# crowsonkb/style_transfer2

Measured on AMD Instinct MI355X. Metric: style-transfer iters/sec @1024px VGG19, higher is better.
Workload: dtype f32; 1 GPU; configs[1]: 1024x1024 single image per GPU, VGG19 to conv5_1, content conv4_2 + 5 style layers, adam fp32, 500 iterations per image; jobs=1, parallelism=independent jobs, 1 per GPU, no collective (replicas)

## Files before the change

### style_transfer2_amd/csrc/conv3x3_winograd.hip

```cpp
#include <hip/hip_runtime.h>
#include <stdint.h>
#include <stdlib.h>
#include <string.h>
#include <type_traits>
#include "st2_kernels.h"
#include "env.h"

namespace st2 {

typedef float f32x16 __attribute__((ext_vector_type(16)));
typedef float f32x4 __attribute__((ext_vector_type(4)));


constexpr int WN_CH = 8;
constexpr int WN_IW = 40;
constexpr int WN_V = 4 * 16 * 64;

size_t wino_pack_floats(int K, int M) { return (size_t)((M + 127) / 128 * 4) * (K / 2) * 1024; }

static void wino_pack(const float* w, int Cout, int Cin, bool dgrad, float* dst)
{
    const int K = dgrad ? Cout : Cin, M = dgrad ? Cin : Cout, nkp = K / 2;
    memset(dst, 0, wino_pack_floats(K, M) * sizeof(float));
    static const double G[4][3] = {{1, 0, 0}, {0.5, 0.5, 0.5}, {0.5, -0.5, 0.5}, {0, 0, 1}};
    for (int m = 0; m < M; ++m)
        for (int k = 0; k < K; ++k) {
            double g[3][3], t[4][3], u[4][4];
            for (int tap = 0; tap < 9; ++tap)
                g[tap / 3][tap % 3] = dgrad ? w[((size_t)k * Cin + m) * 9 + (8 - tap)] : w[((size_t)m * Cin + k) * 9 + tap];
            for (int i = 0; i < 4; ++i)
                for (int j = 0; j < 3; ++j) t[i][j] = G[i][0] * g[0][j] + G[i][1] * g[1][j] + G[i][2] * g[2][j];
            for (int i = 0; i < 4; ++i)
                for (int j = 0; j < 4; ++j) u[i][j] = t[i][0] * G[j][0] + t[i][1] * G[j][1] + t[i][2] * G[j][2];
            const size_t base = ((size_t)(m / 32) * nkp + k / 2) * 1024;
            const int lane = (k & 1) * 32 + (m & 31);
            for (int pos = 0; pos < 16; ++pos)
                dst[base + ((size_t)(pos >> 2) * 64 + lane) * 4 + (pos & 3)] = (float)u[pos >> 2][pos & 3];
        }
}
void pack_wino_weights_fwd(const float* w, int Cout, int Cin, float* dst) { wino_pack(w, Cout, Cin, false, dst); }
void pack_wino_weights_dgrad(const float* w, int Cout, int Cin, float* dst) { wino_pack(w, Cout, Cin, true, dst); }

struct WinoKArgs {
    const float* in; const float4* upack; const float* bias; float* out;
    const float* mask_src; const float* inject;
    int K, M, H, W, nch, tiles_x, tiles_y, n_mtiles, relu;
    unsigned in_bytes, u_bytes;
    float* pool_out; int pool_h, pool_w;
    unsigned char* pool_amap;
    const unsigned char* unpool_amap; unsigned amap_bytes; int ph, pw;
    int splits; float* scratch;
    unsigned long long* stamps;
};

typedef __attribute__((address_space(3))) void* lptr_t;
constexpr unsigned kOOB = 0xffffffffu;

__device__ __forceinline__ float f4c(const float4& v, int i) { return i == 0 ? v.x : i == 1 ? v.y : i == 2 ? v.z : v.w; }

template <int WM, int TG, int DIAG = 0, bool QUAD = true, bool PS = false, bool W8 = false, bool H4 = false, bool UNPOOL = false, bool BIG = false,
          bool NOOUT = false, int EPI = 0>
__device__ __forceinline__ void conv3x3_wino_body(const WinoKArgs& a)
{
    static_assert(EPI == 0 || (QUAD && TG == 1 && !PS && !W8 && !BIG && DIAG == 0), "specialised epilogues: aligned widths, one tile group, four waves, below 4 GiB");
    static_assert(!NOOUT || EPI == 0 || EPI == 2, "no-output builds pool");
    static_assert(!NOOUT || (QUAD && TG == 1 && !PS && !W8 && !UNPOOL && !BIG && DIAG == 0), "no-output builds: the builds that write the arg-max map");
    static_assert(!BIG || (QUAD && TG == 1 && !PS && !W8 && DIAG == 0), "big tensors: aligned widths, one tile group, four waves");
    static_assert(!UNPOOL || (QUAD && TG == 1 && !PS && !W8), "unpool: aligned widths, one tile group, four waves");
    static_assert(H4 || (WM * TG == 4 && (TG == 1 || TG == 2)), "4 waves");
    static_assert(!PS || (WM == 2 && TG == 2), "position split: 2 channel slices x 2 position halves");
    static_assert(!W8 || (WM == 4 && TG == 1 && QUAD && !PS), "eight waves: 4 channel slices x 2 position halves, aligned widths");
    static_assert(!H4 || (WM == 2 && TG == 1 && QUAD && !PS && !W8), "half tile: 2 channel slices x 2 position halves, aligned widths");
    constexpr bool RS = W8 || H4;
    constexpr bool AMAP = QUAD && TG == 1;
    constexpr int NW = W8 ? 8 : 4;
    constexpr int PARTNER = W8 ? 4 : 2;
    constexpr bool SPLIT = PS || RS;
    constexpr int BM = 32 * WM;
    constexpr int PROWS = 4 * TG;
    constexpr int IN_ROWS = PROWS + 2;
    constexpr int IW = QUAD ? WN_IW : 64;
    constexpr int COL0 = QUAD ? 3 : 0;
    constexpr int PLANE = IN_ROWS * IW;
    constexpr int UP_ROWS = PROWS / 2 + 2, UP_COLS = 24;
    constexpr int UP_PLANE = UP_ROWS * UP_COLS;
    constexpr int UP_F = WN_CH * UP_PLANE;
    constexpr int UP_FQ = UP_F / 256, UP_AQ = UP_F / 256;
    static_assert(!UNPOOL || (UP_F % 256 == 0 && NW == 4), "unpool staging is a whole number of wave-DMAs");
    constexpr int N_RAW = UNPOOL ? UP_F + UP_F / 4 : WN_CH * PLANE;
    constexpr int I_PER_WAVE = UNPOOL ? (UP_FQ + UP_AQ + NW - 1) / NW
                             : QUAD ? (N_RAW / 4 + 64 * NW - 1) / (64 * NW) : WN_CH * IN_ROWS / 4;
    constexpr int RAW = UNPOOL ? 1024 : QUAD ? I_PER_WAVE * NW * 256 : N_RAW;
    static_assert(QUAD || (WN_CH * IN_ROWS) % 4 == 0, "rows divide over the four waves");

    __shared__ __attribute__((aligned(16))) float raw_s[2][RAW];
    __shared__ __attribute__((aligned(16))) float v_s[2][TG][WN_V];
    __shared__ __attribute__((aligned(16))) float x8_own[W8 ? 8 * 8 * 64 * 4 : 4];
    static_assert(!H4 || 4 * 8 * 64 * 4 <= 2 * TG * WN_V, "H4: the exchange buffer fits the V images");
    float* const x8_s = H4 ? &v_s[0][0][0] : x8_own;

    const int tid = threadIdx.x;
    const int lane = tid & 63;
    const int wave = __builtin_amdgcn_readfirstlane(tid >> 6);
    const int wave_m = W8 ? (wave & 3) : H4 ? (wave & 1) : wave / TG, wave_g = RS ? 0 : wave % TG;
    const int ph = W8 ? wave >> 2 : H4 ? wave >> 1 : wave_g;

    const int nwg = gridDim.x / a.splits;
    const int split = blockIdx.x / nwg, orig = blockIdx.x - split * nwg;
    const int nch = a.nch / a.splits, c_first = split * nch;
    const int xcd = orig & 7, q = nwg >> 3, r = nwg & 7;
    const int logical = (xcd < r ? xcd * (q + 1) : r * (q + 1) + (xcd - r) * q) + (orig >> 3);
    const int n_pt = a.tiles_x * a.tiles_y;
    const int mt = logical / n_pt;
    const int pt = logical - mt * n_pt;
    const int tx = pt % a.tiles_x;
    const int ty = pt / a.tiles_x;
    const int y0 = ty * PROWS, x0 = tx * 32;
    const unsigned plane = (unsigned)a.H * a.W;
    const int nkp = a.K >> 1;

    const unsigned long long t_begin = DIAG ? __builtin_amdgcn_s_memtime() : 0ull;

    const __amdgpu_buffer_rsrc_t rs_i = __builtin_amdgcn_make_buffer_rsrc((void*)a.in, 0, a.in_bytes, 0x00020000);
    const __amdgpu_buffer_rsrc_t rs_a = __builtin_amdgcn_make_buffer_rsrc((void*)(UNPOOL ? a.unpool_amap : nullptr), 0, UNPOOL ? a.amap_bytes : 0u, 0x00020000);
    const unsigned pplane = UNPOOL ? (unsigned)a.ph * a.pw : 0u;
    unsigned ioff[QUAD ? I_PER_WAVE : 1];
    if (UNPOOL) {
#pragma unroll
        for (int t = 0; t < I_PER_WAVE; ++t) {
            const int piece = wave + NW * t;
            const bool bytes = piece >= UP_FQ;
            const int e = ((bytes ? piece - UP_FQ : piece) * 64 + lane) * 4;
            const int c = e / UP_PLANE;
            const int rem = e - c * UP_PLANE;
            const int rr = rem / UP_COLS;
            const int col = rem - rr * UP_COLS;
            const int gy = (y0 >> 1) - 1 + rr, gx = (x0 >> 1) - 4 + col;
            const bool ok = piece < UP_FQ + UP_AQ && gy >= 0 && gy < a.ph && gx >= 0 && gx + 3 < a.pw;
            ioff[t] = ok ? ((unsigned)((BIG && !bytes ? 0 : c_first * WN_CH) + c) * pplane + (unsigned)gy * a.pw + gx) * (bytes ? 1u : 4u) : kOOB;
        }
    } else if (QUAD) {
#pragma unroll
        for (int t = 0; t < I_PER_WAVE; ++t) {
            const int e = ((wave + NW * t) * 64 + lane) * 4;
            const int c = e / PLANE;
            const int rem = e - c * PLANE;
            const int rr = rem / IW;
            const int col = rem - rr * IW;
            const int gy = y0 - 1 + rr, gx = x0 - 4 + col;
            const bool ok = e < N_RAW && gy >= 0 && gy < a.H && gx >= 0 && gx + 3 < a.W;
            ioff[t] = ok ? ((unsigned)((BIG ? 0 : c_first * WN_CH) + c) * plane + (unsigned)gy * a.W + gx) * 4u : kOOB;
        }
    } else {
        const int gx = x0 - 1 + lane;
        ioff[0] = (lane < 34 && gx >= 0 && gx < a.W) ? (unsigned)gx * 4u : kOOB;
    }
    auto dma_raw = [&](int ch, int buf) {
        const __amdgpu_buffer_rsrc_t rs_c = BIG ? __builtin_amdgcn_make_buffer_rsrc(
            (void*)(a.in + (size_t)(c_first + ch) * WN_CH * (UNPOOL ? pplane : plane)), 0, a.in_bytes, 0x00020000) : rs_i;
        if (UNPOOL) {
#pragma unroll
            for (int t = 0; t < I_PER_WAVE; ++t) {
                const int piece = wave + NW * t;
                if (piece < UP_FQ) {
                    const unsigned vo = (ioff[t] == kOOB || BIG) ? ioff[t] : ioff[t] + (unsigned)ch * WN_CH * pplane * 4u;
                    __builtin_amdgcn_raw_ptr_buffer_load_lds(rs_c, (lptr_t)(raw_s[buf] + piece * 256), 16, vo, 0, 0, 0);
                } else if (piece < UP_FQ + UP_AQ) {
                    const unsigned vo = ioff[t] == kOOB ? kOOB : ioff[t] + (unsigned)ch * WN_CH * pplane;
                    __builtin_amdgcn_raw_ptr_buffer_load_lds(rs_a, (lptr_t)(raw_s[buf] + UP_F + (piece - UP_FQ) * 64), 4, vo, 0, 0, 0);
                }
            }
        } else if (QUAD) {
            const unsigned coff = BIG ? 0u : (unsigned)ch * WN_CH * plane * 4u;
#pragma unroll
            for (int t = 0; t < I_PER_WAVE; ++t) {
                const unsigned vo = ioff[t] == kOOB ? kOOB : ioff[t] + coff;
                __builtin_amdgcn_raw_ptr_buffer_load_lds(rs_c, (lptr_t)(raw_s[buf] + (wave + NW * t) * 256), 16, vo, 0, 0, 0);
            }
        } else {
#pragma unroll
            for (int t = 0; t < I_PER_WAVE; ++t) {
                const int row = wave + 4 * t;
                const int c = row / IN_ROWS, gy = y0 - 1 + (row - c * IN_ROWS);
                const bool row_ok = gy >= 0 && gy < a.H;
                const unsigned base = ((unsigned)((c_first + ch) * WN_CH + c) * plane + (unsigned)(row_ok ? gy : 0) * a.W) * 4u;
                const unsigned vo = (row_ok && ioff[0] != kOOB) ? ioff[0] + base : kOOB;
                __builtin_amdgcn_raw_ptr_buffer_load_lds(rs_i, (lptr_t)(raw_s[buf] + row * 64), 4, vo, 0, 0, 0);
            }
        }
    };

    const int xt = tid & 31, xch = (tid >> 5) & 7;
    const int x_raw = UNPOOL ? xch * UP_PLANE + (xt >> 4) * UP_COLS + (xt & 15) + 3
                             : xch * PLANE + (2 * (xt >> 4)) * IW + 2 * (xt & 15) + COL0;
    const int x_v = (((xch >> 1) * 4) * 64 + (xch & 1) * 32 + xt) * 4;
    float d[TG][16];
    auto pin = [&]() {
#pragma unroll
        for (int g = 0; g < TG; ++g) {
            asm volatile("" : "+v"(d[g][0]), "+v"(d[g][1]), "+v"(d[g][2]), "+v"(d[g][3]), "+v"(d[g][4]), "+v"(d[g][5]), "+v"(d[g][6]), "+v"(d[g][7]));
            asm volatile("" : "+v"(d[g][8]), "+v"(d[g][9]), "+v"(d[g][10]), "+v"(d[g][11]), "+v"(d[g][12]), "+v"(d[g][13]), "+v"(d[g][14]), "+v"(d[g][15]));
        }
    };
    float up_v[UNPOOL ? 9 : 1];
    unsigned up_m[UNPOOL ? 9 : 1];
    auto up_expand = [&]() {
        if constexpr (UNPOOL) {
#pragma unroll
            for (int i = 0; i < 4; ++i)
#pragma unroll
                for (int j = 0; j < 4; ++j) {
                    const int r = (i + 1) >> 1, cc = (j + 1) >> 1;
                    const unsigned want = 4u | (2u * ((i + 1) & 1)) | ((j + 1) & 1);
                    d[0][4 * i + j] = up_m[3 * r + cc] == want ? up_v[3 * r + cc] : 0.f;
                }
        }
    };
    auto xf_read = [&](const float* rp) {
        if constexpr (UNPOOL) {
            const unsigned char* bp = reinterpret_cast<const unsigned char*>(rp - x_raw + UP_F) + x_raw;
#pragma unroll
            for (int r = 0; r < 3; ++r)
#pragma unroll
                for (int cc = 0; cc < 3; ++cc) {
                    up_v[3 * r + cc] = rp[r * UP_COLS + cc];
                    up_m[3 * r + cc] = bp[r * UP_COLS + cc];
                }
            return;
        }
#pragma unroll
        for (int g = 0; g < TG; ++g)
#pragma unroll
            for (int i = 0; i < 4; ++i)
#pragma unroll
                for (int j = 0; j < 4; ++j) d[g][4 * i + j] = rp[(4 * g + i) * IW + j];
    };
    auto xf_math = [&]() {
#pragma unroll
        for (int g = 0; g < TG; ++g) {
            float wv[16];
#pragma unroll
            for (int j = 0; j < 4; ++j) {
                wv[j] = d[g][j] - d[g][8 + j]; wv[4 + j] = d[g][4 + j] + d[g][8 + j];
                wv[8 + j] = d[g][8 + j] - d[g][4 + j]; wv[12 + j] = d[g][4 + j] - d[g][12 + j];
            }
#pragma unroll
            for (int i = 0; i < 4; ++i) {
                d[g][4 * i] = wv[4 * i] - wv[4 * i + 2]; d[g][4 * i + 1] = wv[4 * i + 1] + wv[4 * i + 2];
                d[g][4 * i + 2] = wv[4 * i + 2] - wv[4 * i + 1]; d[g][4 * i + 3] = wv[4 * i + 1] - wv[4 * i + 3];
            }
        }
    };
    auto xf_write = [&](float* vp) {
#pragma unroll
        for (int g = 0; g < TG; ++g)
#pragma unroll
            for (int i = 0; i < 4; ++i)
                *reinterpret_cast<float4*>(vp + g * WN_V + i * 256) = make_float4(d[g][4 * i], d[g][4 * i + 1], d[g][4 * i + 2], d[g][4 * i + 3]);
    };

    const f32x4* up = reinterpret_cast<const f32x4*>(a.upack) + ((size_t)(mt * WM + wave_m) * nkp + 4 * c_first) * 256 + lane;
    constexpr int UQ = SPLIT ? 2 : 4;
    f32x4 ua[4][UQ];
    auto u_fill = [&](int kp) {
#pragma unroll
        for (int g = 0; g < UQ; ++g) ua[kp & 3][g] = up[((size_t)kp * 4 + (SPLIT ? 2 * ph + g : g)) * 64];
        asm volatile("" ::: "memory");
    };
    auto u_pin = [&](int set) {
        if constexpr (SPLIT) asm volatile("" : "+v"(ua[set][0]), "+v"(ua[set][1]));
        else asm volatile("" : "+v"(ua[set][0]), "+v"(ua[set][1]), "+v"(ua[set][2]), "+v"(ua[set][3]));
    };
    constexpr int NACC = RS ? 8 : 16;
    constexpr int NBQ = NACC / 4;
    f32x4 bq[2][NBQ];
    auto b_fetch = [&](int buf, int kpl, int set) {
#pragma unroll
        for (int pg = 0; pg < NBQ; ++pg) {
            const float* vimg = PS ? v_s[buf][pg >> 1] : v_s[buf][wave_g];
            const int quad = PS ? 2 * ph + (pg & 1) : (RS ? 2 * ph + pg : pg);
            bq[set][pg] = *reinterpret_cast<const f32x4*>(vimg + ((kpl * 4 + quad) * 64 + lane) * 4);
        }
    };
    auto b_pin = [&](int set) {
        if constexpr (RS) asm volatile("" : "+v"(bq[set][1]));
        else asm volatile("" : "+v"(bq[set][1]), "+v"(bq[set][2]), "+v"(bq[set][3]));
    };

    f32x16 acc[NACC];
#pragma unroll
    for (int p = 0; p < NACC; ++p)
#pragma unroll
        for (int e = 0; e < 16; ++e) acc[p][e] = 0.f;

    dma_raw(0, 0);
    if (nch > 1) dma_raw(1, 1);
    u_fill(0); u_fill(1); u_fill(2);
    __syncthreads();
    if (!W8 || ph == 0) {
        xf_read(raw_s[0] + x_raw);
        up_expand();
        xf_math();
        xf_write(&v_s[0][0][0] + x_v);
    }
    __syncthreads();
    b_fetch(0, 0, 0);

    unsigned long long t0 = 0, r0 = 0;
    if (DIAG) { t0 = __builtin_amdgcn_s_memtime(); r0 = __builtin_amdgcn_s_memrealtime(); }

    auto chunk = [&](const int c, auto more_t, auto more2_t) {
        constexpr bool MORE = decltype(more_t)::value, MORE2 = decltype(more2_t)::value;
        const int cur = c & 1;
        const bool do_xf = !W8 || ph == ((c + 1) & 1);
#pragma unroll
        for (int kpl = 0; kpl < 4; ++kpl) {
            const int kp = 4 * c + kpl;
            const int set = kpl & 1;
#pragma unroll
            for (int p = 0; p < NACC; ++p) {
                acc[p] = __builtin_amdgcn_mfma_f32_32x32x2f32(ua[kpl][SPLIT ? (p >> 2) & 1 : p >> 2][p & 3], bq[set][p >> 2][p & 3], acc[p], 0, 0, 0);
                if (p == 0) {
                    __builtin_amdgcn_sched_barrier(0);
                    b_pin(set);
                    if (kpl < 3) b_fetch(cur, kpl + 1, set ^ 1);
                    else if (MORE) {
                        if constexpr (SPLIT) asm volatile("s_waitcnt vmcnt(4) lgkmcnt(0)\n\ts_barrier" ::: "memory");
                        else asm volatile("s_waitcnt vmcnt(8) lgkmcnt(0)\n\ts_barrier" ::: "memory");
                        b_fetch(cur ^ 1, 0, 0);
                    }
                    if (MORE || kpl == 0) u_fill(kp + 3);
                    if (MORE && do_xf) {
                        if (kpl == 0) xf_read(raw_s[cur ^ 1] + x_raw);
                        if (kpl == 1) { up_expand(); pin(); xf_math(); pin(); }
                        if (kpl == 2) xf_write(&v_s[cur ^ 1][0][0] + x_v);
                    }
                    if (MORE2 && kpl == 0) dma_raw(c + 2, cur);
                    if (MORE || kpl < 3) u_pin((kpl + 1) & 3);
                    __builtin_amdgcn_sched_barrier(0);
                }
            }
            __builtin_amdgcn_sched_barrier(0);
        }
    };
    {
        using T = std::true_type; using F = std::false_type;
        int c = 0;
        for (; c + 2 < nch; ++c) chunk(c, T{}, T{});
        if (c + 1 < nch) { chunk(c, T{}, F{}); ++c; }
        chunk(c, F{}, F{});
    }

    unsigned long long t_loop_end = 0;
    if (DIAG) {
        const unsigned long long t1 = __builtin_amdgcn_s_memtime(), r1 = __builtin_amdgcn_s_memrealtime();
        t_loop_end = t1;
        if (tid == 0 && a.stamps) { a.stamps[2 * blockIdx.x] = t1 - t0; a.stamps[2 * blockIdx.x + 1] = r1 - r0; }
    }
    float* const xbuf = &v_s[0][0][0];
    auto partial_out = [&](auto grp_t, auto e0_t, int el, float (&y)[4]) {
        constexpr int grp = decltype(grp_t)::value, e0 = decltype(e0_t)::value;
        float t0[4], t1[4];
#pragma unroll
        for (int j = 0; j < 4; ++j) {
            const float ra = acc[(grp * 8 + j) % NACC][e0 + el], rb = acc[(grp * 8 + 4 + j) % NACC][e0 + el];
            if (ph == 0) { t0[j] = ra + rb; t1[j] = rb; }
            else { t0[j] = ra; t1[j] = -ra - rb; }
        }
        y[0] = t0[0] + t0[1] + t0[2]; y[1] = t0[1] - t0[2] - t0[3];
        y[2] = t1[0] + t1[1] + t1[2]; y[3] = t1[1] - t1[2] - t1[3];
    };
    if constexpr (PS) {
        __syncthreads();
#pragma unroll
        for (int e = 0; e < 16; ++e) {
            float y[4];
            if (wave_g == 0) partial_out(std::integral_constant<int, 1>{}, std::integral_constant<int, 0>{}, e, y);
            else partial_out(std::integral_constant<int, 0>{}, std::integral_constant<int, 0>{}, e, y);
            *reinterpret_cast<float4*>(xbuf + ((wave * 16 + e) * 64 + lane) * 4) = make_float4(y[0], y[1], y[2], y[3]);
        }
        __syncthreads();
    }
    if constexpr (RS) {
        if constexpr (H4) __syncthreads();
#pragma unroll
        for (int el = 0; el < 8; ++el) {
            float y[4];
            if (ph == 0) partial_out(std::integral_constant<int, 0>{}, std::integral_constant<int, 8>{}, el, y);
            else partial_out(std::integral_constant<int, 0>{}, std::integral_constant<int, 0>{}, el, y);
            *reinterpret_cast<float4*>(x8_s + ((wave * 8 + el) * 64 + lane) * 4) = make_float4(y[0], y[1], y[2], y[3]);
        }
        __syncthreads();
    }
    auto out_xf = [&](int e, float& y00, float& y01, float& y10, float& y11) {
        if constexpr (RS) {
            float y[4];
            if (ph == 0) partial_out(std::integral_constant<int, 0>{}, std::integral_constant<int, 0>{}, e, y);
            else partial_out(std::integral_constant<int, 0>{}, std::integral_constant<int, 8>{}, e, y);
            const float4 o = *reinterpret_cast<const float4*>(x8_s + (((wave ^ PARTNER) * 8 + e) * 64 + lane) * 4);
            y00 = y[0] + o.x; y01 = y[1] + o.y; y10 = y[2] + o.z; y11 = y[3] + o.w;
        } else if constexpr (PS) {
            float y[4];
            if (wave_g == 0) partial_out(std::integral_constant<int, 0>{}, std::integral_constant<int, 0>{}, e, y);
            else partial_out(std::integral_constant<int, 1>{}, std::integral_constant<int, 0>{}, e, y);
            const float4 o = *reinterpret_cast<const float4*>(xbuf + (((wave ^ 1) * 16 + e) * 64 + lane) * 4);
            y00 = y[0] + o.x; y01 = y[1] + o.y; y10 = y[2] + o.z; y11 = y[3] + o.w;
        } else {
            float tt[2][4];
#pragma unroll
            for (int j = 0; j < 4; ++j) {
                tt[0][j] = acc[j][e] + acc[4 + j][e] + acc[(8 + j) % NACC][e];
                tt[1][j] = acc[4 + j][e] - acc[(8 + j) % NACC][e] - acc[(12 + j) % NACC][e];
            }
            y00 = tt[0][0] + tt[0][1] + tt[0][2]; y01 = tt[0][1] - tt[0][2] - tt[0][3];
            y10 = tt[1][0] + tt[1][1] + tt[1][2]; y11 = tt[1][1] - tt[1][2] - tt[1][3];
        }
    };
  if (!QUAD) {
    const int t31 = lane & 31, khalf = lane >> 5;
    const int gy0 = y0 + 4 * wave_g + 2 * (t31 >> 4), gx = x0 + 2 * (t31 & 15);
    const bool part = a.splits > 1;
    const bool has_bias = !part && a.bias != nullptr, has_mask = !part && a.mask_src != nullptr, has_inj = !part && a.inject != nullptr;
    const bool relu = !part && a.relu;
    float* const outp = part ? a.scratch + (size_t)split * a.M * plane : a.out;
    const bool live = gx < a.W && gy0 < a.H;
    const bool row1 = gy0 + 1 < a.H, col1 = gx + 1 < a.W, wide = (a.W & 1) == 0;
    const int mw = mt * BM + wave_m * 32 + 4 * khalf;
    const unsigned pix0 = live ? (unsigned)gy0 * a.W + gx : 0u, pix1 = (live && row1) ? pix0 + a.W : pix0;
    auto ld2 = [&](const float* base, unsigned off) -> float2 {
        if (wide) return *reinterpret_cast<const float2*>(base + off);
        return make_float2(base[off], col1 ? base[off + 1] : 0.f);
    };
#pragma unroll
    for (int eb = 0; eb < 4; ++eb) {
        const int mb = mw + 8 * eb;
        unsigned off[4];
        float2 mk[4][2], ij[4][2];
        float bs[4];
#pragma unroll
        for (int ee = 0; ee < 4; ++ee) {
            const int m = mb + ee < a.M ? mb + ee : a.M - 1;
            off[ee] = (unsigned)m * plane;
            bs[ee] = has_bias ? a.bias[m] : 0.f;
        }
        if (has_mask) {
#pragma unroll
            for (int ee = 0; ee < 4; ++ee) { mk[ee][0] = ld2(a.mask_src, off[ee] + pix0); mk[ee][1] = ld2(a.mask_src, off[ee] + pix1); }
        }
        if (has_inj) {
#pragma unroll
            for (int ee = 0; ee < 4; ++ee) { ij[ee][0] = ld2(a.inject, off[ee] + pix0); ij[ee][1] = ld2(a.inject, off[ee] + pix1); }
        }
#pragma unroll
        for (int ee = 0; ee < 4; ++ee) {
            const int e = 4 * eb + ee;
            float o[2][2];
            out_xf(e, o[0][0], o[0][1], o[1][0], o[1][1]);
            if (a.pool_out && live && mb + ee < a.M) {
                float pm = o[0][0];
                if (col1) pm = pm > o[0][1] ? pm : o[0][1];
                if (row1) { pm = pm > o[1][0] ? pm : o[1][0]; if (col1) pm = pm > o[1][1] ? pm : o[1][1]; }
                pm += bs[ee];
                if (relu) pm = pm > 0.f ? pm : 0.f;
                a.pool_out[((size_t)(mb + ee) * a.pool_h + (gy0 >> 1)) * a.pool_w + (gx >> 1)] = pm;
            }
#pragma unroll
            for (int i = 0; i < 2; ++i) {
                float o0 = o[i][0] + bs[ee], o1 = o[i][1] + bs[ee];
                if (relu) { o0 = o0 > 0.f ? o0 : 0.f; o1 = o1 > 0.f ? o1 : 0.f; }
                if (has_mask) { o0 = mk[ee][i].x > 0.f ? o0 : 0.f; o1 = mk[ee][i].y > 0.f ? o1 : 0.f; }
                if (has_inj) { o0 += ij[ee][i].x; o1 += ij[ee][i].y; }
                if (live && mb + ee < a.M && (i == 0 || row1)) {
                    float* dst = outp + off[ee] + (i ? pix1 : pix0);
                    if (wide) *reinterpret_cast<float2*>(dst) = make_float2(o0, o1);
                    else { dst[0] = o0; if (col1) dst[1] = o1; }
                }
            }
        }
    }
  } else if constexpr (EPI != 0) {
    constexpr bool E_FWD = EPI == 1 || EPI == 2, E_POOL = EPI == 2, E_MASK = EPI == 3;
    typedef unsigned wn_u32x4 __attribute__((ext_vector_type(4)));
    const int t31 = lane & 31, khalf = lane >> 5;
    const int odd = lane & 1;
    const int gy = y0 + 4 * wave_g + 2 * (t31 >> 4) + odd;
    const int gx4 = x0 + 2 * (t31 & 14);
    const bool live = gx4 < a.W && gy < a.H;
    const int mw = mt * BM + wave_m * 32 + 4 * khalf;
    const unsigned pix = live ? (unsigned)gy * a.W + gx4 : 0u;
    const unsigned out_bytes = (unsigned)a.M * plane * 4u;
    const bool has_inj = a.inject != nullptr;
    const __amdgpu_buffer_rsrc_t rs_o = __builtin_amdgcn_make_buffer_rsrc((void*)a.out, 0, NOOUT ? 0u : out_bytes, 0x00020000);
    const __amdgpu_buffer_rsrc_t rs_mk = __builtin_amdgcn_make_buffer_rsrc((void*)a.mask_src, 0, E_MASK ? out_bytes : 0u, 0x00020000);
    const __amdgpu_buffer_rsrc_t rs_ij = __builtin_amdgcn_make_buffer_rsrc((void*)a.inject, 0, (!E_FWD && has_inj) ? out_bytes : 0u, 0x00020000);
    const __amdgpu_buffer_rsrc_t rs_bs = __builtin_amdgcn_make_buffer_rsrc((void*)a.bias, 0, E_FWD ? (unsigned)a.M * 4u : 0u, 0x00020000);
    const int ty2 = y0 + 4 * wave_g + 2 * (t31 >> 4), tx2 = x0 + 2 * (t31 & 15);
    const bool plive = E_POOL && tx2 < a.W && ty2 < a.H, prow1 = ty2 + 1 < a.H;
    const unsigned pplane = E_POOL ? (unsigned)a.pool_h * a.pool_w : 0u;
    const unsigned ppix = plive ? (unsigned)(ty2 >> 1) * a.pool_w + (tx2 >> 1) : 0u;
    const __amdgpu_buffer_rsrc_t rs_po = __builtin_amdgcn_make_buffer_rsrc((void*)a.pool_out, 0, E_POOL ? (unsigned)a.M * pplane * 4u : 0u, 0x00020000);
    const __amdgpu_buffer_rsrc_t rs_pa = __builtin_amdgcn_make_buffer_rsrc((void*)a.pool_amap, 0, (E_POOL && a.pool_amap) ? (unsigned)a.M * pplane : 0u, 0x00020000);
    constexpr int NEB = RS ? 2 : 4;
#pragma unroll
    for (int ebl = 0; ebl < NEB; ++ebl) {
        const int eb = RS ? 2 * ph + ebl : ebl;
        const int mb = mw + 8 * eb;
        unsigned off[4];
        float mk[E_MASK ? 4 : 1][4], ij[E_FWD ? 1 : 4][4], bs[E_FWD ? 4 : 1];
#pragma unroll
        for (int ee = 0; ee < 4; ++ee) {
            off[ee] = (live && mb + ee < a.M) ? ((unsigned)(mb + ee) * plane + pix) * 4u : kOOB;
            if constexpr (E_FWD) bs[ee] = __builtin_bit_cast(float, __builtin_amdgcn_raw_buffer_load_b32(rs_bs, (mb + ee) * 4, 0, 0));
        }
        if constexpr (E_MASK) {
#pragma unroll
            for (int ee = 0; ee < 4; ++ee) {
                const uint4 v = __builtin_bit_cast(uint4, __builtin_amdgcn_raw_buffer_load_b128(rs_mk, off[ee], 0, 0));
                mk[ee][0] = __builtin_bit_cast(float, v.x); mk[ee][1] = __builtin_bit_cast(float, v.y); mk[ee][2] = __builtin_bit_cast(float, v.z); mk[ee][3] = __builtin_bit_cast(float, v.w);
            }
        }
        if constexpr (!E_FWD) {
#pragma unroll
            for (int ee = 0; ee < 4; ++ee) {
                const uint4 v = __builtin_bit_cast(uint4, __builtin_amdgcn_raw_buffer_load_b128(rs_ij, off[ee], 0, 0));
                ij[ee][0] = __builtin_bit_cast(float, v.x); ij[ee][1] = __builtin_bit_cast(float, v.y); ij[ee][2] = __builtin_bit_cast(float, v.z); ij[ee][3] = __builtin_bit_cast(float, v.w);
            }
        }
#pragma unroll
        for (int ee = 0; ee < 4; ++ee) {
            const int e = 4 * ebl + ee;
            float y00, y01, y10, y11;
            out_xf(e, y00, y01, y10, y11);
            if constexpr (E_POOL) {
                const float b = bs[E_FWD ? ee : 0];
                float pm = y00 > y01 ? y00 : y01;
                const float p1 = y10 > y11 ? y10 : y11, pm2 = pm > p1 ? pm : p1;
                pm = prow1 ? pm2 : pm;
                const float qb = pm + b;
                const unsigned slot = y00 + b == qb ? 0u : (y01 + b == qb ? 1u : (y10 + b == qb ? 2u : 3u));
                const unsigned po = (plive && mb + ee < a.M) ? (unsigned)(mb + ee) * pplane + ppix : kOOB;
                __builtin_amdgcn_raw_buffer_store_b8((unsigned char)(slot | (qb > 0.f ? 4u : 0u)), rs_pa, po, 0, 0);
                pm += b;
                pm = pm > 0.f ? pm : 0.f;
                __builtin_amdgcn_raw_buffer_store_b32(__builtin_bit_cast(unsigned, pm), rs_po, po == kOOB ? kOOB : po * 4u, 0, 0);
            }
            if constexpr (NOOUT) continue;
            const float s0 = odd ? y00 : y10, s1 = odd ? y01 : y11;
            const float r0 = __builtin_bit_cast(float, __builtin_amdgcn_update_dpp(0, __builtin_bit_cast(int, s0), 0xB1, 0xf, 0xf, true));
            const float r1 = __builtin_bit_cast(float, __builtin_amdgcn_update_dpp(0, __builtin_bit_cast(int, s1), 0xB1, 0xf, 0xf, true));
            float o[4];
            o[0] = odd ? r0 : y00; o[1] = odd ? r1 : y01; o[2] = odd ? y10 : r0; o[3] = odd ? y11 : r1;
#pragma unroll
            for (int j = 0; j < 4; ++j) {
                if constexpr (E_FWD) {
                    o[j] += bs[E_FWD ? ee : 0];
                    o[j] = o[j] > 0.f ? o[j] : 0.f;
                } else {
                    if constexpr (E_MASK) o[j] = mk[E_MASK ? ee : 0][j] > 0.f ? o[j] : 0.f;
                    const float oi = o[j] + ij[E_FWD ? 0 : ee][j];
                    o[j] = has_inj ? oi : o[j];
                }
            }
            wn_u32x4 ov;
#pragma unroll
            for (int j = 0; j < 4; ++j) ov[j] = __builtin_bit_cast(unsigned, o[j]);
            __builtin_amdgcn_raw_buffer_store_b128(ov, rs_o, off[ee], 0, 0);
        }
    }
  } else {
    const int t31 = lane & 31, khalf = lane >> 5;
    const int odd = lane & 1;
    const int gy = y0 + 4 * wave_g + 2 * (t31 >> 4) + odd;
    const int gx4 = x0 + 2 * (t31 & 14);
    const bool part = a.splits > 1;
    const bool has_bias = !part && a.bias != nullptr, has_mask = !part && a.mask_src != nullptr, has_inj = !part && a.inject != nullptr;
    const bool relu = !part && a.relu;
    float* const outp = part ? a.scratch + (size_t)split * a.M * plane : a.out;
    const bool live = gx4 < a.W && gy < a.H;
    const int mw = mt * BM + wave_m * 32 + 4 * khalf;
    const unsigned pix = live ? (unsigned)gy * a.W + gx4 : 0u;
    constexpr int NEB = RS ? 2 : 4;
#pragma unroll
    for (int ebl = 0; ebl < NEB; ++ebl) {
        const int eb = RS ? 2 * ph + ebl : ebl;
        const int mb = mw + 8 * eb;
        unsigned off[4];
        float4 mk[4], ij[4];
        float bs[4];
#pragma unroll
        for (int ee = 0; ee < 4; ++ee) {
            const int m = mb + ee < a.M ? mb + ee : a.M - 1;
            off[ee] = (unsigned)m * plane + pix;
            bs[ee] = has_bias ? a.bias[m] : 0.f;
        }
        if (has_mask) {
#pragma unroll
            for (int ee = 0; ee < 4; ++ee) mk[ee] = *reinterpret_cast<const float4*>(a.mask_src + off[ee]);
        }
        if (has_inj) {
#pragma unroll
            for (int ee = 0; ee < 4; ++ee) ij[ee] = *reinterpret_cast<const float4*>(a.inject + off[ee]);
        }
#pragma unroll
        for (int ee = 0; ee < 4; ++ee) {
            const int e = 4 * ebl + ee;
            float y00, y01, y10, y11;
            out_xf(e, y00, y01, y10, y11);
            if (a.pool_out) {
                const int ty2 = y0 + 4 * wave_g + 2 * (t31 >> 4), tx2 = x0 + 2 * (t31 & 15);
                if (tx2 < a.W && ty2 < a.H && mb + ee < a.M) {
                    const size_t po = ((size_t)(mb + ee) * a.pool_h + (ty2 >> 1)) * a.pool_w + (tx2 >> 1);
                    float pm = y00 > y01 ? y00 : y01;
                    if (ty2 + 1 < a.H) { const float p1 = y10 > y11 ? y10 : y11; pm = pm > p1 ? pm : p1; }
                    if constexpr (AMAP) {
                        if (a.pool_amap) {
                            const float qb = pm + bs[ee];
                            const unsigned slot = y00 + bs[ee] == qb ? 0u : (y01 + bs[ee] == qb ? 1u : (y10 + bs[ee] == qb ? 2u : 3u));
                            a.pool_amap[po] = (unsigned char)(slot | (qb > 0.f ? 4u : 0u));
                        }
                    }
                    pm += bs[ee];
                    if (relu) pm = pm > 0.f ? pm : 0.f;
                    a.pool_out[po] = pm;
                }
            }
            if constexpr (NOOUT) continue;
            const float s0 = odd ? y00 : y10, s1 = odd ? y01 : y11;
            const float r0 = __builtin_bit_cast(float, __builtin_amdgcn_update_dpp(0, __builtin_bit_cast(int, s0), 0xB1, 0xf, 0xf, true));
            const float r1 = __builtin_bit_cast(float, __builtin_amdgcn_update_dpp(0, __builtin_bit_cast(int, s1), 0xB1, 0xf, 0xf, true));
            float o[4];
            o[0] = odd ? r0 : y00; o[1] = odd ? r1 : y01; o[2] = odd ? y10 : r0; o[3] = odd ? y11 : r1;
#pragma unroll
            for (int j = 0; j < 4; ++j) {
                o[j] += bs[ee];
                if (relu) o[j] = o[j] > 0.f ? o[j] : 0.f;
            }
            if (has_mask) {
                o[0] = mk[ee].x > 0.f ? o[0] : 0.f; o[1] = mk[ee].y > 0.f ? o[1] : 0.f;
                o[2] = mk[ee].z > 0.f ? o[2] : 0.f; o[3] = mk[ee].w > 0.f ? o[3] : 0.f;
            }
            if (has_inj) { o[0] += ij[ee].x; o[1] += ij[ee].y; o[2] += ij[ee].z; o[3] += ij[ee].w; }
            if (live && mb + ee < a.M) *reinterpret_cast<float4*>(outp + off[ee]) = make_float4(o[0], o[1], o[2], o[3]);
        }
    }
  }
    if (DIAG) {
        asm volatile("s_waitcnt vmcnt(0)" ::: "memory");
        const unsigned long long t2 = __builtin_amdgcn_s_memtime();
        if (tid == 0 && a.stamps && blockIdx.x == 300)
            printf("[wino stamps] block 300: prologue %llu, loop %llu, epilogue (stores drained) %llu cycles\n", t0 - t_begin, t_loop_end - t0, t2 - t_loop_end);
    }
}


__global__ __launch_bounds__(256, 1) void conv3x3_wino_f32_128x128(const WinoKArgs a) { conv3x3_wino_body<4, 1>(a); }
__global__ __launch_bounds__(256, 1) void conv3x3_wino_f32_64x256(const WinoKArgs a) { conv3x3_wino_body<2, 2>(a); }
__global__ __launch_bounds__(256, 1) void conv3x3_wino_f32_128x128_anyw(const WinoKArgs a) { conv3x3_wino_body<4, 1, 0, false>(a); }
__global__ __launch_bounds__(256, 1) void conv3x3_wino_f32_64x256_anyw(const WinoKArgs a) { conv3x3_wino_body<2, 2, 0, false>(a); }
__global__ __launch_bounds__(256, 1) void conv3x3_wino_f32_ps64x256(const WinoKArgs a) { conv3x3_wino_body<2, 2, 0, true, true>(a); }
__global__ __launch_bounds__(256, 1) void conv3x3_wino_f32_ps64x256_stamped(const WinoKArgs a) { conv3x3_wino_body<2, 2, 1, true, true>(a); }
__global__ __launch_bounds__(512, 2) void conv3x3_wino_f32_w8_128x128(const WinoKArgs a) { conv3x3_wino_body<4, 1, 0, true, false, true>(a); }
__global__ __launch_bounds__(512, 2) void conv3x3_wino_f32_w8_128x128_stamped(const WinoKArgs a) { conv3x3_wino_body<4, 1, 1, true, false, true>(a); }
__global__ __launch_bounds__(256, 2) void conv3x3_wino_f32_h4_64x128(const WinoKArgs a) { conv3x3_wino_body<2, 1, 0, true, false, false, true>(a); }
__global__ __launch_bounds__(256, 2) void conv3x3_wino_f32_h4_64x128_stamped(const WinoKArgs a) { conv3x3_wino_body<2, 1, 1, true, false, false, true>(a); }
__global__ __launch_bounds__(256, 1) void conv3x3_wino_f32_128x128_unpool(const WinoKArgs a) { conv3x3_wino_body<4, 1, 0, true, false, false, false, true>(a); }
__global__ __launch_bounds__(256, 2) void conv3x3_wino_f32_h4_64x128_unpool(const WinoKArgs a) { conv3x3_wino_body<2, 1, 0, true, false, false, true, true>(a); }
__global__ __launch_bounds__(256, 1) void conv3x3_wino_f32_128x128_noout(const WinoKArgs a) { conv3x3_wino_body<4, 1, 0, true, false, false, false, false, false, true>(a); }
__global__ __launch_bounds__(256, 2) void conv3x3_wino_f32_h4_64x128_noout(const WinoKArgs a) { conv3x3_wino_body<2, 1, 0, true, false, false, true, false, false, true>(a); }
#define ST2_WINO_EPI(NAME, BOUNDS, ...) __global__ __launch_bounds__(256, BOUNDS) void NAME(const WinoKArgs a) { conv3x3_wino_body<__VA_ARGS__>(a); }
ST2_WINO_EPI(conv3x3_wino_f32_128x128_fwd, 1, 4, 1, 0, true, false, false, false, false, false, false, 1)
ST2_WINO_EPI(conv3x3_wino_f32_128x128_pool, 1, 4, 1, 0, true, false, false, false, false, false, false, 2)
ST2_WINO_EPI(conv3x3_wino_f32_128x128_poolonly, 1, 4, 1, 0, true, false, false, false, false, false, true, 2)
ST2_WINO_EPI(conv3x3_wino_f32_128x128_dgm, 1, 4, 1, 0, true, false, false, false, false, false, false, 3)
ST2_WINO_EPI(conv3x3_wino_f32_128x128_dg, 1, 4, 1, 0, true, false, false, false, false, false, false, 4)
ST2_WINO_EPI(conv3x3_wino_f32_128x128_unpool_dgm, 1, 4, 1, 0, true, false, false, false, true, false, false, 3)
ST2_WINO_EPI(conv3x3_wino_f32_h4_64x128_fwd, 2, 2, 1, 0, true, false, false, true, false, false, false, 1)
ST2_WINO_EPI(conv3x3_wino_f32_h4_64x128_pool, 2, 2, 1, 0, true, false, false, true, false, false, false, 2)
ST2_WINO_EPI(conv3x3_wino_f32_h4_64x128_poolonly, 2, 2, 1, 0, true, false, false, true, false, false, true, 2)
ST2_WINO_EPI(conv3x3_wino_f32_h4_64x128_dgm, 2, 2, 1, 0, true, false, false, true, false, false, false, 3)
ST2_WINO_EPI(conv3x3_wino_f32_h4_64x128_dg, 2, 2, 1, 0, true, false, false, true, false, false, false, 4)
ST2_WINO_EPI(conv3x3_wino_f32_h4_64x128_unpool_dgm, 2, 2, 1, 0, true, false, false, true, true, false, false, 3)
#undef ST2_WINO_EPI
__global__ __launch_bounds__(256, 1) void conv3x3_wino_f32_128x128_big(const WinoKArgs a) { conv3x3_wino_body<4, 1, 0, true, false, false, false, false, true>(a); }
__global__ __launch_bounds__(256, 2) void conv3x3_wino_f32_h4_64x128_big(const WinoKArgs a) { conv3x3_wino_body<2, 1, 0, true, false, false, true, false, true>(a); }
__global__ __launch_bounds__(256, 1) void conv3x3_wino_f32_128x128_unpool_big(const WinoKArgs a) { conv3x3_wino_body<4, 1, 0, true, false, false, false, true, true>(a); }
__global__ __launch_bounds__(256, 2) void conv3x3_wino_f32_h4_64x128_unpool_big(const WinoKArgs a) { conv3x3_wino_body<2, 1, 0, true, false, false, true, true, true>(a); }
__global__ __launch_bounds__(256, 1) void conv3x3_wino_f32_128x128_stamped(const WinoKArgs a) { conv3x3_wino_body<4, 1, 1>(a); }
__global__ __launch_bounds__(256, 1) void conv3x3_wino_f32_64x256_stamped(const WinoKArgs a) { conv3x3_wino_body<2, 2, 1>(a); }

__global__ __launch_bounds__(256) void wino_combine_k(const float* __restrict__ scratch, int splits, const float* __restrict__ bias, int relu,
                                                      const float* __restrict__ mask_src, const float* __restrict__ inject,
                                                      float* __restrict__ out, int M, unsigned plane)
{
    const size_t n4 = (size_t)M * plane / 4, per = (size_t)M * plane;
    for (size_t i = (size_t)blockIdx.x * 256 + threadIdx.x; i < n4; i += (size_t)gridDim.x * 256) {
        float4 v = *reinterpret_cast<const float4*>(scratch + 4 * i);
        for (int sp = 1; sp < splits; ++sp) {
            const float4 w = *reinterpret_cast<const float4*>(scratch + sp * per + 4 * i);
            v.x += w.x; v.y += w.y; v.z += w.z; v.w += w.w;
        }
        if (bias) { const float b = bias[(4 * i) / plane]; v.x += b; v.y += b; v.z += b; v.w += b; }
        if (relu) { v.x = v.x > 0.f ? v.x : 0.f; v.y = v.y > 0.f ? v.y : 0.f; v.z = v.z > 0.f ? v.z : 0.f; v.w = v.w > 0.f ? v.w : 0.f; }
        if (mask_src) {
            const float4 m = *reinterpret_cast<const float4*>(mask_src + 4 * i);
            v.x = m.x > 0.f ? v.x : 0.f; v.y = m.y > 0.f ? v.y : 0.f; v.z = m.z > 0.f ? v.z : 0.f; v.w = m.w > 0.f ? v.w : 0.f;
        }
        if (inject) { const float4 j = *reinterpret_cast<const float4*>(inject + 4 * i); v.x += j.x; v.y += j.y; v.z += j.z; v.w += j.w; }
        *reinterpret_cast<float4*>(out + 4 * i) = v;
    }
}

hipError_t launch_wino_combine(const float* scratch, int splits, const float* bias, int relu, const float* mask_src, const float* inject,
                               float* out, int M, int H, int W, hipStream_t s)
{
    if (((size_t)H * W) % 4 != 0) return hipErrorInvalidValue;
    const size_t n4 = (size_t)M * H * W / 4;
    const unsigned grid = (unsigned)((n4 + 255) / 256 < 2048 ? (n4 + 255) / 256 : 2048);
    wino_combine_k<<<grid, 256, 0, s>>>(scratch, splits, bias, relu, mask_src, inject, out, M, (unsigned)(H * W));
    return hipGetLastError();
}
// ... 150 lines not shown
```

Baseline: 141.0 it/s.

## Prefetch Winograd epilogue bias/mask/inject loads under final MFMA chunk

Moves the epilogue's global loads of bias, ReLU mask and injected gradient out of the per-block epilogue loop. Part of them are issued during the last K chunk, interleaved with its MFMAs, and the rest right after the loop, before the output transform. This hides their memory latency behind compute instead of stalling each epilogue block. In exchange it keeps all prefetched values live in registers at once, which raises VGPR pressure and could spill or lower occupancy. Inline-asm pins are added to keep the accumulators in AGPRs.

```diff
diff --git a/style_transfer2_amd/csrc/conv3x3_winograd.hip b/style_transfer2_amd/csrc/conv3x3_winograd.hip
--- a/style_transfer2_amd/csrc/conv3x3_winograd.hip
+++ b/style_transfer2_amd/csrc/conv3x3_winograd.hip
@@ -57,6 +57,56 @@
 constexpr unsigned kOOB = 0xffffffffu;
 
 __device__ __forceinline__ float f4c(const float4& v, int i) { return i == 0 ? v.x : i == 1 ? v.y : i == 2 ? v.z : v.w; }
+
+template <int EPI, bool RS> struct WinoEpiOps {
+    static constexpr bool E_FWD = EPI == 1 || EPI == 2, E_MASK = EPI == 3;
+    static constexpr int NEB = RS ? 2 : 4;
+    static constexpr int NG = E_MASK ? 2 * NEB : NEB;
+    static constexpr int UNDER = NG < 4 ? NG : 4;
+    int mw, dm0, odd;
+    bool live, has_inj;
+    unsigned row0, plane4, out_bytes;
+    float mk[E_MASK ? NEB : 1][E_MASK ? 4 : 1][4], ij[E_FWD ? 1 : NEB][E_FWD ? 1 : 4][4], bs[E_FWD ? NEB : 1][E_FWD ? 4 : 1];
+
+    __device__ __forceinline__ void init(const WinoKArgs& a, int lane, int yw, int x0, int m0, int ph, unsigned plane)
+    {
+        odd = lane & 1;
+        const int gy = yw + 2 * ((lane & 31) >> 4) + odd;
+        const int gx4 = x0 + 2 * (lane & 14);
+        live = gx4 < a.W && gy < a.H;
+        mw = m0 + 4 * (lane >> 5);
+        dm0 = RS ? 16 * ph : 0;
+        has_inj = a.inject != nullptr;
+        plane4 = plane * 4u;
+        out_bytes = (unsigned)a.M * plane4;
+        row0 = ((unsigned)mw * plane + (live ? (unsigned)gy * a.W + gx4 : 0u)) * 4u;
+    }
+    __device__ __forceinline__ unsigned row_off(const WinoKArgs& a, int ebl, int ee) const
+    {
+        const int dm = dm0 + 8 * ebl + ee;
+        return (live & (mw + dm < a.M)) ? row0 + (unsigned)dm * plane4 : kOOB;
+    }
+    __device__ __forceinline__ void load(const WinoKArgs& a, int g)
+    {
+        const int ebl = E_MASK ? g >> 1 : g;
+        const bool mask = E_MASK && (g & 1) == 0;
+        const __amdgpu_buffer_rsrc_t rs = E_FWD ? __builtin_amdgcn_make_buffer_rsrc((void*)a.bias, 0, (unsigned)a.M * 4u, 0x00020000)
+                                        : mask ? __builtin_amdgcn_make_buffer_rsrc((void*)a.mask_src, 0, out_bytes, 0x00020000)
+                                               : __builtin_amdgcn_make_buffer_rsrc((void*)a.inject, 0, has_inj ? out_bytes : 0u, 0x00020000);
+#pragma unroll
+        for (int ee = 0; ee < 4; ++ee) {
+            if constexpr (E_FWD) {
+                bs[ebl][ee] = __builtin_bit_cast(float, __builtin_amdgcn_raw_buffer_load_b32(rs, (mw + dm0 + 8 * ebl + ee) * 4, 0, 0));
+            } else {
+                const uint4 v = __builtin_bit_cast(uint4, __builtin_amdgcn_raw_buffer_load_b128(rs, row_off(a, ebl, ee), 0, 0));
+                float (&d4)[4] = mask ? mk[E_MASK ? ebl : 0][E_MASK ? ee : 0] : ij[ebl][ee];
+                d4[0] = __builtin_bit_cast(float, v.x); d4[1] = __builtin_bit_cast(float, v.y); d4[2] = __builtin_bit_cast(float, v.z); d4[3] = __builtin_bit_cast(float, v.w);
+            }
+        }
+        asm volatile("" ::: "memory");
+    }
+};
+template <bool RS> struct WinoEpiOps<0, RS> {};
 
 template <int WM, int TG, int DIAG = 0, bool QUAD = true, bool PS = false, bool W8 = false, bool H4 = false, bool UNPOOL = false, bool BIG = false,
           bool NOOUT = false, int EPI = 0>
@@ -309,6 +359,9 @@
     unsigned long long t0 = 0, r0 = 0;
     if (DIAG) { t0 = __builtin_amdgcn_s_memtime(); r0 = __builtin_amdgcn_s_memrealtime(); }
 
+    WinoEpiOps<EPI, RS> eo;
+    if constexpr (EPI != 0) eo.init(a, lane, y0 + 4 * wave_g, x0, mt * BM + wave_m * 32, ph, plane);
+
     auto chunk = [&](const int c, auto more_t, auto more2_t) {
         constexpr bool MORE = decltype(more_t)::value, MORE2 = decltype(more2_t)::value;
         const int cur = c & 1;
@@ -330,6 +383,12 @@
                         b_fetch(cur ^ 1, 0, 0);
                     }
                     if (MORE || kpl == 0) u_fill(kp + 3);
+                    if constexpr (EPI != 0) {
+                        if constexpr (!MORE) {
+                            constexpr int UNDER = WinoEpiOps<EPI, RS>::UNDER;
+                            if (kpl >= 4 - UNDER) eo.load(a, kpl - (4 - UNDER));
+                        }
+                    }
                     if (MORE && do_xf) {
                         if (kpl == 0) xf_read(raw_s[cur ^ 1] + x_raw);
                         if (kpl == 1) { up_expand(); pin(); xf_math(); pin(); }
@@ -349,6 +408,16 @@
         for (; c + 2 < nch; ++c) chunk(c, T{}, T{});
         if (c + 1 < nch) { chunk(c, T{}, F{}); ++c; }
         chunk(c, F{}, F{});
+    }
+    if constexpr (EPI != 0) {
+        if constexpr (!RS && EPI == 2) {
+#pragma unroll
+            for (int p = 0; p < NACC; ++p) asm volatile("" : "+a"(acc[p]));
+        }
+#pragma unroll
+        for (int g = WinoEpiOps<EPI, RS>::UNDER; g < WinoEpiOps<EPI, RS>::NG; ++g) eo.load(a, g);
+        asm volatile("" : "+v"(eo.row0));
+        __builtin_amdgcn_sched_barrier(0);
     }
 
     unsigned long long t_loop_end = 0;
@@ -480,51 +549,22 @@
     }
   } else if constexpr (EPI != 0) {
     constexpr bool E_FWD = EPI == 1 || EPI == 2, E_POOL = EPI == 2, E_MASK = EPI == 3;
+    constexpr int NEB = RS ? 2 : 4;
     typedef unsigned wn_u32x4 __attribute__((ext_vector_type(4)));
-    const int t31 = lane & 31, khalf = lane >> 5;
-    const int odd = lane & 1;
-    const int gy = y0 + 4 * wave_g + 2 * (t31 >> 4) + odd;
-    const int gx4 = x0 + 2 * (t31 & 14);
-    const bool live = gx4 < a.W && gy < a.H;
-    const int mw = mt * BM + wave_m * 32 + 4 * khalf;
-    const unsigned pix = live ? (unsigned)gy * a.W + gx4 : 0u;
-    const unsigned out_bytes = (unsigned)a.M * plane * 4u;
-    const bool has_inj = a.inject != nullptr;
-    const __amdgpu_buffer_rsrc_t rs_o = __builtin_amdgcn_make_buffer_rsrc((void*)a.out, 0, NOOUT ? 0u : out_bytes, 0x00020000);
-    const __amdgpu_buffer_rsrc_t rs_mk = __builtin_amdgcn_make_buffer_rsrc((void*)a.mask_src, 0, E_MASK ? out_bytes : 0u, 0x00020000);
-    const __amdgpu_buffer_rsrc_t rs_ij = __builtin_amdgcn_make_buffer_rsrc((void*)a.inject, 0, (!E_FWD && has_inj) ? out_bytes : 0u, 0x00020000);
-    const __amdgpu_buffer_rsrc_t rs_bs = __builtin_amdgcn_make_buffer_rsrc((void*)a.bias, 0, E_FWD ? (unsigned)a.M * 4u : 0u, 0x00020000);
+    const int t31 = lane & 31;
+    const __amdgpu_buffer_rsrc_t rs_o = __builtin_amdgcn_make_buffer_rsrc((void*)a.out, 0, NOOUT ? 0u : eo.out_bytes, 0x00020000);
     const int ty2 = y0 + 4 * wave_g + 2 * (t31 >> 4), tx2 = x0 + 2 * (t31 & 15);
     const bool plive = E_POOL && tx2 < a.W && ty2 < a.H, prow1 = ty2 + 1 < a.H;
     const unsigned pplane = E_POOL ? (unsigned)a.pool_h * a.pool_w : 0u;
     const unsigned ppix = plive ? (unsigned)(ty2 >> 1) * a.pool_w + (tx2 >> 1) : 0u;
     const __amdgpu_buffer_rsrc_t rs_po = __builtin_amdgcn_make_buffer_rsrc((void*)a.pool_out, 0, E_POOL ? (unsigned)a.M * pplane * 4u : 0u, 0x00020000);
     const __amdgpu_buffer_rsrc_t rs_pa = __builtin_amdgcn_make_buffer_rsrc((void*)a.pool_amap, 0, (E_POOL && a.pool_amap) ? (unsigned)a.M * pplane : 0u, 0x00020000);
-    constexpr int NEB = RS ? 2 : 4;
 #pragma unroll
     for (int ebl = 0; ebl < NEB; ++ebl) {
-        const int eb = RS ? 2 * ph + ebl : ebl;
-        const int mb = mw + 8 * eb;
-        unsigned off[4];
-        float mk[E_MASK ? 4 : 1][4], ij[E_FWD ? 1 : 4][4], bs[E_FWD ? 4 : 1];
-#pragma unroll
-        for (int ee = 0; ee < 4; ++ee) {
-            off[ee] = (live && mb + ee < a.M) ? ((unsigned)(mb + ee) * plane + pix) * 4u : kOOB;
-            if constexpr (E_FWD) bs[ee] = __builtin_bit_cast(float, __builtin_amdgcn_raw_buffer_load_b32(rs_bs, (mb + ee) * 4, 0, 0));
-        }
-        if constexpr (E_MASK) {
-#pragma unroll
-            for (int ee = 0; ee < 4; ++ee) {
-                const uint4 v = __builtin_bit_cast(uint4, __builtin_amdgcn_raw_buffer_load_b128(rs_mk, off[ee], 0, 0));
-                mk[ee][0] = __builtin_bit_cast(float, v.x); mk[ee][1] = __builtin_bit_cast(float, v.y); mk[ee][2] = __builtin_bit_cast(float, v.z); mk[ee][3] = __builtin_bit_cast(float, v.w);
-            }
-        }
-        if constexpr (!E_FWD) {
-#pragma unroll
-            for (int ee = 0; ee < 4; ++ee) {
-                const uint4 v = __builtin_bit_cast(uint4, __builtin_amdgcn_raw_buffer_load_b128(rs_ij, off[ee], 0, 0));
-                ij[ee][0] = __builtin_bit_cast(float, v.x); ij[ee][1] = __builtin_bit_cast(float, v.y); ij[ee][2] = __builtin_bit_cast(float, v.z); ij[ee][3] = __builtin_bit_cast(float, v.w);
-            }
+        const int mb = eo.mw + eo.dm0 + 8 * ebl;
+        if constexpr (!RS && !E_POOL) {
+#pragma unroll
+            for (int p = 0; p < NACC; ++p) asm volatile("" : "+a"(acc[p]));
         }
 #pragma unroll
         for (int ee = 0; ee < 4; ++ee) {
@@ -532,7 +572,7 @@
             float y00, y01, y10, y11;
             out_xf(e, y00, y01, y10, y11);
             if constexpr (E_POOL) {
-                const float b = bs[E_FWD ? ee : 0];
+                const float b = eo.bs[E_FWD ? ebl : 0][E_FWD ? ee : 0];
                 float pm = y00 > y01 ? y00 : y01;
                 const float p1 = y10 > y11 ? y10 : y11, pm2 = pm > p1 ? pm : p1;
                 pm = prow1 ? pm2 : pm;
@@ -545,27 +585,28 @@
                 __builtin_amdgcn_raw_buffer_store_b32(__builtin_bit_cast(unsigned, pm), rs_po, po == kOOB ? kOOB : po * 4u, 0, 0);
             }
             if constexpr (NOOUT) continue;
-            const float s0 = odd ? y00 : y10, s1 = odd ? y01 : y11;
+            const float s0 = eo.odd ? y00 : y10, s1 = eo.odd ? y01 : y11;
             const float r0 = __builtin_bit_cast(float, __builtin_amdgcn_update_dpp(0, __builtin_bit_cast(int, s0), 0xB1, 0xf, 0xf, true));
             const float r1 = __builtin_bit_cast(float, __builtin_amdgcn_update_dpp(0, __builtin_bit_cast(int, s1), 0xB1, 0xf, 0xf, true));
             float o[4];
-            o[0] = odd ? r0 : y00; o[1] = odd ? r1 : y01; o[2] = odd ? y10 : r0; o[3] = odd ? y11 : r1;
+            o[0] = eo.odd ? r0 : y00; o[1] = eo.odd ? r1 : y01; o[2] = eo.odd ? y10 : r0; o[3] = eo.odd ? y11 : r1;
 #pragma unroll
             for (int j = 0; j < 4; ++j) {
                 if constexpr (E_FWD) {
-                    o[j] += bs[E_FWD ? ee : 0];
+                    o[j] += eo.bs[E_FWD ? ebl : 0][E_FWD ? ee : 0];
                     o[j] = o[j] > 0.f ? o[j] : 0.f;
                 } else {
-                    if constexpr (E_MASK) o[j] = mk[E_MASK ? ee : 0][j] > 0.f ? o[j] : 0.f;
-                    const float oi = o[j] + ij[E_FWD ? 0 : ee][j];
-                    o[j] = has_inj ? oi : o[j];
+                    if constexpr (E_MASK) o[j] = eo.mk[E_MASK ? ebl : 0][E_MASK ? ee : 0][j] > 0.f ? o[j] : 0.f;
+                    const float oi = o[j] + eo.ij[E_FWD ? 0 : ebl][E_FWD ? 0 : ee][j];
+                    o[j] = eo.has_inj ? oi : o[j];
                 }
             }
             wn_u32x4 ov;
 #pragma unroll
             for (int j = 0; j < 4; ++j) ov[j] = __builtin_bit_cast(unsigned, o[j]);
-            __builtin_amdgcn_raw_buffer_store_b128(ov, rs_o, off[ee], 0, 0);
-        }
+            __builtin_amdgcn_raw_buffer_store_b128(ov, rs_o, eo.row_off(a, ebl, ee), 0, 0);
+        }
+        __builtin_amdgcn_sched_barrier(0);
     }
   } else {
     const int t31 = lane & 31, khalf = lane >> 5;
```

After: 142.7 it/s (median of 6 runs). 1.3% higher.
